# yamrom/smash-paper

Measured on AMD Instinct MI355X. Metric: reads/sec mapped+binned (hg19, 150 bp) at 1/2/4/8 MI355X; bit-exact bin counts, higher is better.
Workload: dtype u8/u64 (integer); 1 GPU; C3 hg19-shaped, 50 M x 150 bp SMASH reads per rank (25 M pairs, one run in batches), sample_bins/50000; genome=hg19, index_words=packed (SA / ISA hints, DESIGN section 3), genome_bp=3095693983, text_N=6191388016, pairs_per_rank=25000000, read_len=150, batch_pairs=12500000, bins=50000, parallelism=single GPU

## Files before the change

smash-paper_amd/csrc/mam.hip:

```cpp
#include "common.hpp"
#include "mam_device.hpp"
#include "mam_sm.hpp"

#include <algorithm>
#include <cstdio>
#include <cstdlib>
#include <vector>
#include <cstring>

namespace smash {
namespace {

template <class IdxT, int BLOCK, bool PLAIN>
__global__ __launch_bounds__(BLOCK) void k_mam(
    DevIndex<IdxT> x, const uint8_t *__restrict__ seqs, uint64_t stride,
    const uint16_t *__restrict__ lens, uint32_t len0, uint64_t n_reads,
    uint32_t min_len, uint64_t *__restrict__ out, uint32_t cap,
    uint32_t *__restrict__ n_out, uint32_t row, unsigned long long *work) {
  extern __shared__ uint8_t lds[];
  uint8_t *P = lds + threadIdx.x * row;
  for (;;) {
    const uint64_t r = atomicAdd(work, 1ull);
    if (r >= n_reads) break;
    const uint32_t L = lens ? lens[r] : len0;
// ... 77 lines not shown
    SMASH_HIP(hipMemcpy(ws, c.wave_stats, 128 * 8, hipMemcpyDeviceToHost));
    SMASH_HIP(hipFree(c.iters));
    SMASH_HIP(hipFree(c.wave_stats));
    std::vector<uint32_t> srt(hv);
    std::sort(srt.begin(), srt.end());
    double sum = 0;
    for (uint32_t v : hv) sum += v;
    auto q = [&](double f) { return srt[std::min<size_t>(srt.size() - 1, size_t(f * srt.size()))]; };
    std::fprintf(stderr,
                 "[k_mam_sm] reads %llu blocks %llu (%d/CU) row %u words: lane-iterations/read mean %.1f "
                 "p50 %u p90 %u p99 %u p99.9 %u max %u; wave-iterations %llu, active lanes/iteration %.2f\n",
                 (unsigned long long)n_reads, (unsigned long long)blocks, per_cu, c.w_row, sum / n_reads,
                 q(0.5), q(0.9), q(0.99), q(0.999), srt.back(), ws[0],
                 double(ws[1]) / double(ws[0] ? ws[0] : 1));
    static const char *names[] = {"EXIT", "NEW", "ALU", "COPY", "BM", "KT", "IDX", "BYTE", "CMP",
                                  "USCAN", "EXL", "EXR", "EXB"};
    static const char *idx_ops[] = {"SAPOS", "SAPOS2", "SCAN_SA", "ISAJ", "NS_SA2", "NS_ISA2",
                                    "TD_SA2", "TD_SA"};
    static const char *byte_ops[] = {"TD_T2", "TD_T", "LM"};
    std::fprintf(stderr, "[k_mam_sm] lane-iterations per read by state:");
    for (int k = 0; k < 13; ++k)
      if (ws[2 + k]) std::fprintf(stderr, " %s %.1f", names[k], double(ws[2 + k]) / n_reads);
    for (int k = 0; k < 8; ++k)
      if (ws[18 + k]) std::fprintf(stderr, " IDX.%s %.1f", idx_ops[k], double(ws[18 + k]) / n_reads);
    for (int k = 0; k < 3; ++k)
      if (ws[34 + k]) std::fprintf(stderr, " BYTE.%s %.1f", byte_ops[k], double(ws[34 + k]) / n_reads);
    for (int k = 0; k < 2; ++k)
      if (ws[42 + k]) std::fprintf(stderr, " CMP.%s %.1f", k ? "SCAN" : "EXT", double(ws[42 + k]) / n_reads);
    std::fprintf(stderr, "\n");
    static const char *regions[] = {
        "consume", "S_ALU", "S_COPY", "S_BM", "S_KT", "S_IDX", "S_BYTE", "S_CMP", "S_USCAN",
        "S_EX", "A_BS", "A_BS_DONE", "A_XL_DONE", "A_RUN_DONE", "A_CHAIN_DONE", "A_EXPAND",
        "A_AFTER", "A_TOP", "A_TRAV", "A_DONE", "TOP.!clean", "TOP.codes1", "TOP.codes2",
        "TOP.kt", "TOP.filter", "TOP.kcache", "dma", "rowbad"};
    std::fprintf(stderr, "[k_mam_sm] wave iterations running each region (%%):");
    for (int k = 0; k < 28; ++k)
      if (ws[64 + k])
        std::fprintf(stderr, " %s %.1f", regions[k], 100.0 * double(ws[64 + k]) / double(ws[0] ? ws[0] : 1));
    std::fprintf(stderr, "\n");
  }
  return SMASH_OK;
}

template <class IdxT>
int launch_sm(const smash_index *ix, uint32_t min_len, const uint8_t *seqs,
              uint64_t stride, const uint16_t *lens, uint32_t len,
              uint64_t n_reads, uint64_t *out, uint32_t cap, uint32_t *n_out,
              hipStream_t s, bool sync_check, const SearchWs *ws) {
  constexpr int B = kSmBlock;
  const uint32_t glen = !lens ? len : ws && ws->geom_len ? ws->geom_len : 255u;
  const sm::Geom g = sm::make_geom(glen);
  const bool direct = !lens && search_direct(seqs, stride, len);
  const uint64_t need = direct ? 0 : n_reads * g.chunks * 16;
  uint32_t *rec = ws ? reinterpret_cast<uint32_t *>(ws->rec) : nullptr;
  if (ws && need > ws->rec_bytes) {
    set_error("k_mam_sm: search workspace too small");
    return SMASH_ERR_ARG;
  }
  if (!ws && need > ix->rec_bytes) {
    SMASH_HIP(hipStreamSynchronize(s));
    if (ix->d_rec) SMASH_HIP(hipFree(ix->d_rec));
    ix->d_rec = nullptr;
    ix->rec_bytes = 0;
    const uint64_t bytes = need + need / 4;
    SMASH_HIP(hipMalloc(&ix->d_rec, bytes));
    ix->rec_bytes = bytes;
  }
  if (!ws) rec = ix->d_rec;
  const uint32_t ga = sm::prep_groups(glen);
// ... 217 lines not shown
```

smash-paper_amd/csrc/mam_sm.hpp:

```cpp
#pragma once
#include "mam_device.hpp"

#ifndef PAD_KEEP
#define PAD_KEEP(x) asm volatile("" : "+v"(x))
#endif
#ifndef SM_KNOB
#define SM_KNOB(field, dflt) (dflt)
#endif
#ifndef SM_HOOK_BM
#define SM_HOOK_BM(mode, a1, a2)
#endif
#ifndef SM_HOOK_F
#define SM_HOOK_F(j, bits)
#endif
#ifndef SM_HOOK_BS
#define SM_HOOK_BS(size, depth)
#endif
#ifndef SM_HOOK_CMPBS
#define SM_HOOK_CMPBS(begin, sp, off)
#endif
#ifndef SM_HOOK_RUN
#define SM_HOOK_RUN(begin, kind, ext_l, ext_r)
#endif
#ifndef SM_HOOK_BYTE
#define SM_HOOK_BYTE(pos)
#endif
#ifndef SM_HOOK_PARK
#define SM_HOOK_PARK(a)
#endif
#ifndef SM_LOAD16
#define SM_LOAD16(a) ::smash::sm::load16u(a)
#endif
#ifndef SM_LOAD16ST
#define SM_LOAD16ST(a, st) SM_LOAD16(a)
#endif
#ifndef SM_LOADPF16
#define SM_LOADPF16(a) ::smash::sm::load16u(a)
#endif
#ifndef SM_LOADIDX
#define SM_LOADIDX(p, i) uint64_t((p)[i])
#endif
#ifndef SM_HOOK_PF
#define SM_HOOK_PF(a)
#endif
#ifndef SM_PERM
#define SM_PERM(s0, s1, sel) __builtin_amdgcn_perm(s0, s1, sel)
#endif

#define SM_REGION(k)                                                              \
  do {                                                                            \
    if (STATS) {                                                                  \
      const uint64_t am_ = __ballot(1);                                           \
      if (lane == uint32_t(__builtin_ctzll(am_))) atomicAdd(c.wave_stats + 64 + (k), 1ull); \
    }                                                                             \
  } while (0)

#ifndef SM_DMA_ROW
#define SM_DMA_ROW(dst, src, n, lane) ::smash::sm::dma_row(dst, src, n, lane)
#endif

namespace smash {
namespace sm {

#ifdef SM_DMA_ROW_HOST
__device__ __forceinline__ uint4 load16u(uint64_t a) {
  uint4 v;
  __builtin_memcpy(&v, reinterpret_cast<const uint8_t *>(a), 16);
  return v;
}
#else
typedef uint32_t sm_u32x4 __attribute__((ext_vector_type(4)));
typedef sm_u32x4 sm_u32x4_u __attribute__((aligned(1)));
typedef __attribute__((address_space(1))) const sm_u32x4_u glb_block16_t;
__device__ __forceinline__ uint4 load16u(uint64_t a) {
  const sm_u32x4 b = *reinterpret_cast<glb_block16_t *>(a);
  return make_uint4(b.x, b.y, b.z, b.w);
}
#endif

#ifndef SM_DMA_ROW_HOST
typedef __attribute__((address_space(3))) void lds_void_t;
typedef __attribute__((address_space(1))) const void glb_void_t;
__device__ __forceinline__ void dma_row(uint32_t *dst, const uint4 *src, uint32_t n, uint32_t lane) {
  if (lane < n)
    __builtin_amdgcn_global_load_lds((glb_void_t *)(src + lane), (lds_void_t *)dst, 16, 0, 0);
}
#endif

// ... 143 lines not shown
        const uint32_t b = (w >> (8 * j)) & 0xFF;
        const bool live = i0 + j < L;
        if (!live) w &= ~(0xFFu << (8 * j));
        const uint32_t good = (b == 'a' ? ia : 0u) | (b == 'c' ? ic : 0u) |
                              (b == 'g' ? ig : 0u) | (b == 't' ? iu : 0u);
        bw |= uint32_t(live && !good) << (4 * k + j);
      }
      w8[k] = 8 * gi + k < g.w_raw ? w : 0u;
    }
  }
  o[gi] = bw;
  uint32_t *raw = o + 4 * g.c_bad;
  if (8 * gi + 8 <= g.w_row) {
    reinterpret_cast<uint4 *>(raw + 8 * gi)[0] = make_uint4(w8[0], w8[1], w8[2], w8[3]);
    reinterpret_cast<uint4 *>(raw + 8 * gi)[1] = make_uint4(w8[4], w8[5], w8[6], w8[7]);
  } else {
#pragma unroll
    for (uint32_t k = 0; k < 8; ++k)
      if (8 * gi + k < g.w_row) raw[8 * gi + k] = w8[k];
  }
  if (gi == ga - 1) {
    for (uint32_t k = ga; k < 4 * g.c_bad; ++k) o[k] = 0;
    for (uint32_t k = 8 * ga; k < g.w_row; ++k) raw[k] = 0;
  }
}

inline uint32_t prep_groups(uint32_t max_len) { return (max_len + 31) / 32; }

enum : uint32_t { S_EXIT = 0, S_NEW, S_ALU, S_COPY, S_BM, S_KT, S_IDX, S_BYTE, S_CMP, S_USCAN,
                  S_EXL, S_EXR, S_EXB };
enum : uint32_t { O_SAPOS, O_SAPOS2, O_BS_SA, O_ISAJ, O_NS_SA2, O_NS_ISA2 };
enum : uint32_t { O_EXT = 0, O_BS };
enum : uint32_t { A_NONE = 0, A_BSP, A_BS, A_BS_DONE, A_XL_DONE, A_RUN_DONE, A_CHAIN_DONE,
                  A_EXPAND, A_AFTER, A_TOP, A_TRAV, A_DONE, A_EMIT, A_EXS };
enum : uint32_t { BS_INSERT = 0, BS_LEFT, BS_RIGHT };

__device__ __forceinline__ uint64_t lo64(const uint4 &v) { return uint64_t(v.x) | (uint64_t(v.y) << 32); }
__device__ __forceinline__ uint64_t hi64(const uint4 &v) { return uint64_t(v.z) | (uint64_t(v.w) << 32); }
__device__ __forceinline__ uint32_t dword_at(const uint4 &v, uint32_t i) {
  return i == 0 ? v.x : i == 1 ? v.y : i == 2 ? v.z : v.w;
}
__device__ __forceinline__ uint32_t byte_at(const uint4 &v, uint32_t o) {
  return (dword_at(v, o >> 2) >> (8 * (o & 3))) & 0xFF;
}
__device__ __forceinline__ uint64_t bytes8_at(const uint4 &v, uint32_t o) {
  const uint64_t lo = lo64(v), hi = hi64(v);
  if (o == 0) return lo;
  if (o < 8) return (lo >> (8 * o)) | (hi << (64 - 8 * o));
  if (o == 8) return hi;
  return hi >> (8 * (o - 8));
}
__device__ __forceinline__ uint32_t agree_block(const uint4 &v, uint32_t o, const uint8_t *P,
                                                uint32_t poff, uint32_t lim) {
  uint32_t k = agree8(bytes8_at(v, o), lds_load8(P, poff), lim < 8 ? lim : 8u);
  if (k == 8 && lim > 8) k += agree8(bytes8_at(v, o + 8), lds_load8(P, poff + 8), lim - 8);
  return k;
}
template <class F>
__device__ __forceinline__ uint32_t byte_mask(const uint4 &v, F f) {
  uint32_t m = 0;
#pragma unroll
  for (uint32_t i = 0; i < 16; ++i) {
    const uint32_t b = (dword_at(v, i >> 2) >> (8 * (i & 3))) & 0xFF;
    m |= uint32_t(f(b, i)) << i;
  }
  return m;
}
// ... 192 lines not shown
}

#ifndef SM_GEO_WPS
#define SM_GEO_WPS 1
#endif
template <class IdxT, int BLOCK, bool CHECK, bool STATS, bool PK = false, int GEO = 0>
__global__ __launch_bounds__(BLOCK, GEO ? SM_GEO_WPS : 1) void k_mam_sm(const Ctx<IdxT> c) {
  static_assert(GEO == 0 || (GEO >= 21 && GEO <= 255), "GEO is 0 or the read length");
  const uint32_t gK = GEO ? 16u : c.K, gMin = GEO ? 20u : c.min_len, gB = GEO ? 18u : c.B;
  const uint32_t gRow = GEO ? geo_row(GEO) : c.w_row, gLen0 = GEO ? uint32_t(GEO) : c.len0;
  const uint32_t gDirect = GEO ? 1u : c.direct, gPad = GEO ? 0u : c.pad, gMh = GEO ? 1u : c.mhint;
  const uint32_t gLogN = GEO ? 33u : c.logN, gCap = GEO ? uint32_t(GEO) - 19u : c.cap;
  const uint16_t *const gLens = GEO ? nullptr : c.lens;
  static_assert(!PK || sizeof(IdxT) == 8, "packed words are 8-byte elements");
  constexpr uint64_t PM = PK ? kPkPosMask : ~0ull;
  extern __shared__ uint32_t ldsw[];
  const uint64_t it0 = c.in_text[0], it1 = c.in_text[1], it2 = c.in_text[2], it3 = c.in_text[3];
  auto in_text = [&](uint32_t b) {
    const uint64_t w = b < 64 ? it0 : b < 128 ? it1 : b < 192 ? it2 : it3;
    return ((w >> (b & 63)) & 1ull) != 0;
  };
  const uint64_t N = c.N;
  uint32_t *row = ldsw + threadIdx.x * gRow;
  const uint8_t *P = reinterpret_cast<const uint8_t *>(row);
  const uint32_t lane = threadIdx.x & 63;
  const uint32_t row_live = 4 * lane < gLen0 ? (gLen0 - 4 * lane < 4 ? gLen0 - 4 * lane : 4u) : 0u;

  uint64_t q_next = 0, q_end = 0;
  uint32_t st = S_NEW, op = 0, pend = A_NONE;
  uint64_t addr = 0, addr2 = 0;
  uint32_t fl = 0;
  FlagRef need2{fl, 0};
  uint64_t rd = 0;
  uint32_t L = 0, nem = 0;
  Bad bad{0, 0, 0, 0, 0, 0, 0, 0};
  uint32_t prefix = 0, depth = 0;
  uint64_t start = 0, end = 0, pos = 0;
  FlagRef have_pos{fl, 1};
  uint64_t lo = 0, hi = 0, bpos = 0, sp = 0, m = 0, bi = 0, es = 0, ee = 0;
  uint64_t &c0 = bpos, &c1 = sp;
  uint32_t lL = 0, lR = 0, best = 0, lc = 0, cbase = 0, cap = 0, bsm = 0, nblk = 0;
  FlagRef hit{fl, 2}, bm2{fl, 3}, skip_f{fl, 4}, xrun{fl, 5};
  FlagRef rdone{fl, 6};
  uint32_t fm = 0;
  uint32_t fk = 0, kp = 0, fj = 0, kx = 0xFFFFFFFFu;
  uint64_t klo = 1, khi = 0;
  FlagRef fdead{fl, 11};
  FlagRef ktr_set{fl, 7};
  FlagRef clean{fl, 8};
  FlagRef pf{fl, 9}, pfr{fl, 10};
  FlagRef xls{fl, 12}, xl1{fl, 13}, xrs{fl, 14}, xr1{fl, 15};
  FlagRef em{fl, 16};
  uint32_t dch = 0, j = 0, thresh = 0, xd = 0;
  uint32_t it = 0;
  uint64_t w_iters = 0, w_active = 0;
  auto uscan_start = [&](uint64_t p, uint32_t d) {
    dch = d; j = 1;
    addr = reinterpret_cast<uint64_t>(c.U + p + 1);
    addr2 = addr + 16;
    need2 = SM_KNOB(u32, 1u) && d - 1 > 16;
    st = S_USCAN;
  };
  auto bs_decide = [&](bool ranout, uint32_t pb, uint32_t tb) {
    bool left;
    if (bsm == BS_INSERT) {
      left = ranout || int8_t(pb) < int8_t(tb);
      if (lc > best) { best = lc; bpos = sp; bi = m; }
    } else {
      left = (lc >= cap) == (bsm == BS_LEFT);
    }
    if (left) { hi = m; lR = lc; }
    else { lo = m + 1; lL = lc; }
  };
  auto bs_probe = [&]() -> bool {
    SM_HOOK_CMPBS(true, sp, cbase + lc);
    const uint32_t o = cbase + lc;
    if (PK && ((sp >> kPkPosBits) & 7u) != 5u && o - gK < kPkWindow) {
      const uint32_t rem = cap - lc, nav = gK + kPkWindow - o;
      const uint32_t lim = rem < nav ? rem : nav;
      const uint64_t win = pk_window(sp) >> (8 * (o - gK));
      const uint32_t k = agree8(win, lds_load8(P, prefix + o), lim);
      lc += k;
      if (k < lim || k == rem) {
        SM_HOOK_CMPBS(false, sp, cbase + lc);
        bs_decide(k == rem, k == rem ? 0u : uint32_t(P[prefix + o + k]),
                  uint32_t(win >> (8 * (k & 7))) & 0xFFu);
        pf = false; pfr = false; need2 = false;
        return true;
      }
    }
    addr = reinterpret_cast<uint64_t>(c.T + (sp & PM) + cbase + lc);
    addr2 = ia(c.SA, (lo + m) >> 1);
    need2 = SM_KNOB(pf, 1u) && lo < m;
    pfr = SM_KNOB(pf, 1u) && m + 1 < hi;
    pf = SM_KNOB(pf, 1u) != 0;
    st = S_CMP; op = O_BS;
    return false;
  };
  auto lblock = [&](uint64_t e) { return reinterpret_cast<uint64_t>(c.L8 + (e >= 15 ? e - 15 : 0)); };
  auto ex_start = [&](uint64_t lb, uint64_t hb, bool ls, bool rs) {
    const bool l = !ls && es > lb, r = !rs && ee < hb;
    nblk = 0;
    rdone = !r;
    addr = l ? lblock(es) : reinterpret_cast<uint64_t>(c.L8 + ee + 1);
    addr2 = reinterpret_cast<uint64_t>(c.L8 + ee + 1);
    need2 = l && r;
    st = l && r ? S_EXB : l ? S_EXL : S_EXR;
    return l || r;
  };

  auto isa_hints = [&](uint64_t wl, uint64_t wr) {
    const uint32_t d = depth;
    xls = pk_below(wl, 40, d) || (pk_above(wl, 40, d) && pk_below(wl, 33, d));
    xl1 = !pk_below(wl, 40, d);
    xrs = pk_below(wr, 47, d) || (pk_above(wr, 47, d) && pk_below(wr, 54, d));
    xr1 = !pk_below(wr, 47, d);
  };

  for (;;) {
    const uint64_t newm = __ballot(st == S_NEW);
    const uint32_t need = uint32_t(__popcll(newm));
    const uint64_t avail = q_end - q_next;
    const uint64_t live = __ballot(st != S_EXIT);
    if (live == 0) break;
    if (STATS) { w_iters += 1; w_active += __popcll(live); }
    const uint32_t st_ld = S_COPY + gDirect;
    if (CHECK && st >= st_ld &&
        (addr < c.lo || addr >= c.hi || (need2 && (addr2 < c.lo || addr2 >= c.hi)))) {
      if (atomicAdd(c.viol, 1ull) == 0) {
        c.viol[1] = st; c.viol[2] = op; c.viol[3] = addr; c.viol[4] = need2 ? addr2 : 0;
// ... 42 lines not shown
          cm &= cm - 1;
          const uint32_t w = row_live ? ldsw[ln * gRow + lane] : 0u;
          const uint32_t nib = row_live ? bad_nibble(w, c.bad_tab_lo, c.bad_tab_hi, row_live) : 0u;
          if (__ballot(nib != 0)) {
            uint32_t x = nib << (4 * (lane & 7));
            x |= __shfl_xor(x, 1, 64);
            x |= __shfl_xor(x, 2, 64);
            x |= __shfl_xor(x, 4, 64);
            const uint32_t m0 = __shfl(x, 0, 64), m1 = __shfl(x, 8, 64), m2 = __shfl(x, 16, 64),
                           m3 = __shfl(x, 24, 64), m4 = __shfl(x, 32, 64), m5 = __shfl(x, 40, 64),
                           m6 = __shfl(x, 48, 64), m7 = __shfl(x, 56, 64);
            if (lane == ln) bad = Bad{m0, m1, m2, m3, m4, m5, m6, m7};
          }
        }
#endif
      }
    }
    bool fresh = false;
    if (newm) {
      if (take) base = __shfl(base, int(__builtin_ctzll(newm)), 64);
      if (st == S_NEW) {
        fresh = true;
        const uint32_t r = uint32_t(__popcll(newm & ((1ull << lane) - 1)));
        rd = r < avail ? q_next + r : base + (r - avail);
        if (rd >= c.n_reads) {
          st = S_EXIT;
        } else {
          L = gLens ? gLens[rd] : gLen0;
          addr = reinterpret_cast<uint64_t>(c.rec + rd * c.chunks);
          addr2 = addr + 16;
          need2 = !gDirect && c.c_bad > 1;
          pf = false; pfr = false;
          bad = Bad{0, 0, 0, 0, 0, 0, 0, 0};
          st = S_COPY;
        }
      }
      if (take) { q_next = base + (need - avail); q_end = base + take; }
      else q_next += need;
      uint64_t fm_ = __ballot(fresh && st == S_COPY);
      if (fm_) SM_REGION(26);
      while (fm_) {
        const uint32_t ln = uint32_t(__builtin_ctzll(fm_));
        fm_ &= fm_ - 1;
        const uint64_t rl = __shfl(rd, int(ln), 64);
        if (gDirect)
          SM_DMA_ROW(ldsw + ln * gRow, c.rows + rl * (gRow >> 2), gRow >> 2, lane);
        else
          SM_DMA_ROW(ldsw + ln * gRow, c.rec + rl * c.chunks + c.c_bad, c.chunks - c.c_bad, lane);
      }
    }
    if (st < S_ALU || fresh) continue;
    if (STATS) {
      ++it;
      atomicAdd(c.wave_stats + 2 + (st == S_IDX ? 16 + op : st == S_CMP ? 40 + op : st), 1ull);
    }
#ifdef SM_TRACE
    if (st != S_COPY)
      printf("it %u st %u op %u prefix %u depth %u [%llu,%llu] pos %llu hp %d\n", it, st, op, prefix,
             depth, (unsigned long long)start, (unsigned long long)end, (unsigned long long)pos,
             int(have_pos));
#endif
    const uint32_t ao = st >= S_BYTE ? 0u : uint32_t(addr) & 15;
    uint32_t a = A_NONE;
    SM_REGION(0);
    uint32_t mv = 0, mv2 = 0;
    if (st >= S_USCAN) {
      const bool us = st == S_USCAN;
      const uint32_t base = us ? dch - j - 1 : xd - 1;
      mv = thr_mask(v, base, us);
      mv2 = thr_mask(v2, us ? base - 16 : base, us);
    }

    switch (st) {
      case S_ALU:
        SM_REGION(1);
        a = pend;
        break;
      case S_COPY: {
        SM_REGION(2);
        if (!gDirect) {
          bad.w0 = v.x; bad.w1 = v.y; bad.w2 = v.z; bad.w3 = v.w;
          bad.w4 = v2.x; bad.w5 = v2.y; bad.w6 = v2.z; bad.w7 = v2.w;
        }
        need2 = false;
        prefix = 0; depth = 0; start = 0; end = N - 1; have_pos = false; nem = 0;
        skip_f = false; fm = 0; ktr_set = false;
        fk = 0; kp = 0; kx = 0xFFFFFFFFu; fdead = false;
        clean = (bad.w0 | bad.w1 | bad.w2 | bad.w3 | bad.w4 | bad.w5 | bad.w6 | bad.w7) == 0;
        a = A_TOP;
        break;
      }
      case S_BM: {
        SM_REGION(3);
        const bool two = need2;
        need2 = false;
        if (SM_KNOB(bm_dual, 3u) == 3) {
          const uint32_t nb = 2 * (gK + 4);
          auto entry_bits = [&](const uint4 &e, uint64_t cc) {
            const uint64_t f48 = kt_filter(lo64(e), hi64(e));
            const uint32_t l1 = uint32_t(cc >> (nb - 2)) & 3, l0 = uint32_t(cc >> (nb - 4)) & 3;
            const uint32_t r1 = uint32_t(cc >> 2) & 3, r2 = uint32_t(cc) & 3;
            return (uint32_t(f48 >> (32 + 4 * l1 + l0)) & 1u) |
                   ((uint32_t(f48 >> (16 + 4 * l0 + r1)) & 1u) << 1) |
                   ((uint32_t(f48 >> (4 * r1 + r2)) & 1u) << 2);
          };
          const uint32_t bits = entry_bits(v, c0);
          SM_HOOK_F(fj, bits);
          fk |= (7u << fj) | (bits << (16 + fj));
          fdead = bits != 7u;
          if (two) {
            const uint32_t bits2 = entry_bits(v2, c1);
            SM_HOOK_F(fj + 3, bits2);
            fk |= (7u << (fj + 3)) | (bits2 << (19 + fj));
            fdead = fdead || bits2 != 7u;
          }
          kx = kp + fj + 2;
          klo = lo64(v) & kKtMask;
          khi = hi64(v) & kKtMask;
          a = A_TOP;
          break;
        }
        const uint64_t cc = bm2 ? c0 : c1;
        const bool pa = (lo64(v) >> (40 + (cc & 15))) & 1ull;
        const bool pb = !SM_KNOB(bm_dual, 3u) || ((lo64(v2) >> (40 + (c0 & 15))) & 1ull);
        if (SM_KNOB(bm_dual, 3u) == 2) {
          const uint32_t D = gMin - gB;
          const uint32_t fm0 = fm;
          SM_HOOK_BM(fm, pa, pb);
          uint32_t adv = 0, nfm = 0;
          bool pass = false;
          if (fm == 0) {
            if (!pa) { adv = D + 1; nfm = 1; }
            else if (!pb) adv = 1;
            else pass = true;
          } else if (fm == 1) {
            if (!pa && !pb) { adv = 2 * D + 2; nfm = 1; }
            else if (!pa) { adv = D + 1; nfm = 2; }
            else nfm = 2;
          } else {
            if (!pb) adv = 2;
            else if (!pa) adv = 1;
            else pass = true;
          }
          if (pass) {
            skip_f = true; fm = 1;
            m = (fm0 == 0 ? c0 : c1) >> (2 * (gB - gK));
            ktr_set = true;
          } else {
            fm = nfm;
            if (adv) { depth = 0; start = 0; end = N - 1; have_pos = false; prefix += adv; }
          }
          a = A_TOP;
        } else if (!pa && !bm2) {
          depth = 0; start = 0; end = N - 1; have_pos = false;
          prefix += gMin - gB + 1;
          a = A_TOP;
        } else if (!pa || !pb) {
          depth = 0; start = 0; end = N - 1; have_pos = false; ++prefix; a = A_TOP;
        } else if (!bm2 && !SM_KNOB(bm_dual, 3u)) {
          bm2 = true;
          addr = reinterpret_cast<uint64_t>(c.KT + 2 * (c0 >> 4));
        } else {
          skip_f = true;
          a = A_TOP;
        }
        break;
      }
      case S_KT: {
        SM_REGION(4);
        const uint64_t l0 = lo64(v) & kKtMask, h0 = hi64(v) & kKtMask;
        if (l0 <= h0) { depth = gK; start = l0; end = h0; have_pos = false; }
        a = A_TRAV;
        break;
      }
      case S_IDX: {
        SM_REGION(5);
        const uint64_t iv = idx_val<IdxT>(v, ao);
        const uint64_t iv2 = idx_val<IdxT>(v2, uint32_t(addr2) & 15);
        if (PK && (op == O_ISAJ || op == O_NS_ISA2)) isa_hints(iv, op == O_ISAJ ? iv : iv2);
        if (op == O_SAPOS || op == O_SAPOS2) {
          pos = iv; have_pos = true;
          a = op == O_SAPOS ? A_TRAV : A_AFTER;
        } else if (op == O_BS_SA) {
          sp = iv;
          a = A_BSP;
        } else if (op == O_ISAJ) {
          start = end = iv & PM; have_pos = false;
          a = A_EXPAND;
        } else if (op == O_NS_SA2) {
          addr = ia(c.ISA, (iv & PM) + 1); addr2 = ia(c.ISA, (iv2 & PM) + 1);
          op = O_NS_ISA2;
        } else {
          start = iv & PM; end = iv2 & PM; need2 = false;
          ++prefix; have_pos = false;
          if (depth == 0) { start = 0; end = N - 1; a = A_TOP; }
          else a = A_EXPAND;
        }
        break;
      }
      case S_BYTE: {
        SM_REGION(6);
        SM_HOOK_BYTE(pos & PM);
        em = P[prefix - 1] != uint8_t(byte_at(v, ao));
        a = A_EMIT;
        break;
      }
      case S_CMP: {
        SM_REGION(7);
        const bool tn2 = need2 && !pf;
        const uint32_t off = prefix + (op == O_BS ? cbase : depth) + lc;
        const uint32_t rem = op == O_BS ? cap - lc : L - off;
        const uint32_t lim = rem < 16 ? rem : 16u;
        uint32_t k = agree_block(v, 0, P, off, lim);
        if (tn2 && k == lim && k < rem) {
          const uint32_t lim2 = rem - k < 16 ? rem - k : 16u;
          k += agree_block(v2, 0, P, off + k, lim2);
        }
        const uint32_t got = tn2 ? (rem < 32 ? rem : 32u) : lim;
        const bool had_pf = pf;
        pf = false; pfr = false;
        lc += k;
        if (k == got && k < rem) {
          addr += k;
          addr2 = addr + 16;
          need2 = rem - k > 16;
        } else if (op == O_EXT) {
          need2 = false;
          depth += lc; lc = 0;
          a = A_AFTER;
        } else {
          SM_HOOK_CMPBS(false, sp, cbase + lc);
          need2 = false;
          const uint32_t tbyte = k < 16 ? byte_at(v, k) : byte_at(v2, k - 16);
          bs_decide(k == rem, k == rem ? 0u : uint32_t(P[off + k]), tbyte);
          const bool left = hi == m;
          if (had_pf && lo < hi) {
            m = (lo + hi) >> 1;
            SM_HOOK_PF(ia(c.SA, m));
            sp = left ? idx_val<IdxT>(v2, uint32_t(m * sizeof(IdxT)) & 15) : v3;
            lc = lL < lR ? lL : lR;
            a = A_BSP;
          } else {
            a = A_BS;
          }
        }
        break;
      }
      case S_USCAN: {
        SM_REGION(8);
        bool fin = false;
#pragma unroll
        for (uint32_t h = 0; h < 2; ++h) {
          if (fin || (h == 1 && !need2)) break;
          const uint32_t D = dch - j;
          const uint32_t lim = D < 16 ? D : 16u;
          const uint32_t inr = (1u << lim) - 1;
          const uint32_t hm = (h ? mv2 : mv) & inr;
          if (hm) {
            j += uint32_t(__builtin_ctz(hm)); hit = true; fin = true;
          } else {
            j += lim;
            if (j >= dch) { hit = false; fin = true; }
          }
        }
        if (fin) {
          need2 = false;
          a = A_CHAIN_DONE;
        } else {
          addr += need2 ? 32 : 16;
          addr2 = addr + 16;
          need2 = SM_KNOB(u32, 1u) && dch - j > 16;
        }
        break;
      }
      case S_EXL:
      case S_EXR:
      case S_EXB: {
        SM_REGION(9);
        const uint64_t lb = xrun ? start : 0, hb = xrun ? end : N - 1;
        auto side = [&](uint32_t mask, uint32_t o, bool left, bool &more) {
          const uint64_t room = left ? es - lb : hb - ee;
          const uint32_t w = left ? o + 1 : 16 - o;
          const uint32_t lim = room < uint64_t(w) ? uint32_t(room) : w;
          const uint32_t below = ~mask & 0xFFFFu;
          const uint32_t win = left ? (((1u << lim) - 1) << (o + 1 - lim)) : (((1u << lim) - 1) << o);
          const uint32_t sm = below & win;
          const uint32_t k = sm ? (left ? o - (31 - __builtin_clz(sm)) : uint32_t(__builtin_ctz(sm)) - o)
                                : lim;
          more = !sm && uint64_t(k) < room;
          return k;
        };
        bool moreL = false, moreR = false;
        if (st != S_EXR)
          es -= side(mv, uint32_t(es - (addr - reinterpret_cast<uint64_t>(c.L8))), true, moreL);
        if (st != S_EXL) {
          const bool b2 = st == S_EXB;
          ee += side(b2 ? mv2 : mv, 0u, false, moreR);
          if (b2) rdone = !moreR;
        }
        need2 = false;
        const bool left = st != S_EXR;
        const bool more = left ? moreL : moreR;
        if (!more) {
          a = left ? A_XL_DONE : A_RUN_DONE;
        } else if (++nblk < SM_KNOB(lin_blocks, 8u)) {
          addr = left ? lblock(es) : reinterpret_cast<uint64_t>(c.L8 + ee + 1);
          st = left ? S_EXL : S_EXR;
        } else {
          bsm = left ? BS_LEFT : BS_RIGHT;
          if (left) { lo = lb; hi = es; lL = 0; lR = cap; }
          else { lo = ee + 1; hi = hb + 1; lL = cap; lR = 0; }
          a = A_BS;
        }
        break;
      }
      default:
        break;
    }

    if (gPad) {
      uint32_t x = uint32_t(addr);
      for (uint32_t k = 0; k < gPad; ++k) {
        x += k;
        PAD_KEEP(x);
      }
    }

    if (a == A_BSP) {
      a = bs_probe() ? A_BS : A_NONE;
    }
    if (a == A_BS) {
      SM_REGION(10);
      if (lo < hi) {
        m = (lo + hi) >> 1;
        lc = lL < lR ? lL : lR;
        addr = ia(c.SA, m);
        st = S_IDX; op = O_BS_SA;
        a = A_NONE;
      } else {
        a = A_BS_DONE;
      }
    }
    if (a == A_BS_DONE) {
      SM_REGION(11);
      lc = 0;
      if (bsm == BS_LEFT) {
        es = lo;
        a = A_XL_DONE;
      } else if (bsm == BS_RIGHT) {
        ee = lo - 1;
        a = A_RUN_DONE;
      } else if (best == 0) {
        a = A_AFTER;
      } else {
        xd = depth + best; xrun = true;
        cbase = depth; cap = best;
        es = bi; ee = bi;
        SM_HOOK_RUN(true, 1, 0, 0);
        xls = PK && pk_below(bpos, 36, xd); xrs = PK && pk_below(bpos, 43, xd);
        a = A_EXS;
      }
    }
    if (a == A_EXPAND) {
      SM_REGION(15);
      thresh = 2u * depth * gLogN;
      xd = depth; xrun = false;
      cbase = 0; cap = depth;
      es = start; ee = end;
      SM_HOOK_RUN(true, 0, 0, 0);
      if (PK) {
        if (xls && xl1) es = start - 1;
        if (xrs && xr1) ee = end + 1;
      }
      a = A_EXS;
    }
    if (a == A_EXS) {
      a = ex_start(xrun ? start : 0, xrun ? end : N - 1, xls, xrs) ? A_NONE : A_RUN_DONE;
    }
    if (a == A_XL_DONE) {
      SM_REGION(12);
      const uint64_t hb = xrun ? end : N - 1;
      nblk = 0;
      if (!xrun && start - es >= thresh) {
        SM_HOOK_RUN(false, 0, start - es, 99);
        depth = 0; start = 0; end = N - 1; have_pos = false;
        a = A_TOP;
      } else if (ee < hb && !rdone) {
        addr = reinterpret_cast<uint64_t>(c.L8 + ee + 1);
        st = S_EXR;
        a = A_NONE;
      } else {
        a = A_RUN_DONE;
      }
    }
    if (a == A_RUN_DONE) {
      SM_REGION(13);
      SM_HOOK_RUN(false, xrun ? 1 : 0, xrun ? bi - es : start - es, xrun ? ee - bi : ee - end);
      if (xrun) {
        start = es; end = ee; depth = xd; pos = bpos; have_pos = start == end;
        a = A_AFTER;
      } else if ((start - es) + (ee - end) >= thresh) {
        depth = 0; start = 0; end = N - 1; have_pos = false;
        a = A_TOP;
      } else {
        start = es; end = ee;
        a = A_TOP;
      }
    }
    if (a == A_CHAIN_DONE) {
      SM_REGION(14);
      prefix += j;
      if (!hit) {
        depth = 0; start = 0; end = N - 1; have_pos = false;
        a = A_TOP;
      } else {
        depth = dch - j;
        addr = ia(c.ISA, (pos & PM) + j);
        st = S_IDX; op = O_ISAJ;
        a = A_NONE;
      }
    }
    if (a == A_TOP) {
      SM_REGION(17);
      uint32_t kpos = ~0u;
      const uint32_t bp0 = prefix;
      uint64_t bwin = 0;
      if (!clean) bwin = bad.bits64(prefix);
      auto badw = [&](uint32_t p, uint32_t n) {
        return uint32_t(bwin >> (p - bp0)) & ((1u << n) - 1u);
      };
      bool proceed = skip_f || depth >= gMin;
      const bool ktr = skip_f && ktr_set;
      skip_f = false; ktr_set = false;
      if (prefix >= L || (!proceed && prefix + gMin > L)) {
        a = A_DONE;
      } else if (!proceed) {
        SM_REGION(24);
        int32_t kb = -1;
        const uint32_t B = gB;
        const uint32_t D = gMin - B;
        if (!clean) {
          SM_REGION(20);
          kb = bad.last(prefix, gMin);
          while (kb >= 0 && in_text(P[kb]))
            kb = bad.last(prefix, uint32_t(kb) - prefix);
        }
        if (kb >= 0) {
          depth = 0; start = 0; end = N - 1; have_pos = false;
          prefix = uint32_t(kb) + 1;
          fm = 0;
        } else if (SM_KNOB(bm_dual, 3u) == 3) {
          if (B != gK + 2 || B > gMin || D + 3 > 16) {
            proceed = true;
          } else {
            const uint32_t sh = prefix - kp;
            uint32_t kn = sh < 16 ? (fk & 0xFFFFu) >> sh : 0u;
// ... 85 lines not shown
          if (kx == prefix) {
            SM_REGION(25);
            if (klo <= khi) { depth = gK; start = klo; end = khi; have_pos = false; }
            a = A_TRAV;
          } else {
            SM_REGION(23);
            if (ktr) addr = reinterpret_cast<uint64_t>(c.KT + 2 * m);
            else kpos = prefix;
            st = S_KT;
            a = A_NONE;
          }
        } else {
          a = A_TRAV;
        }
      }
      if (kpos != ~0u) {
        const uint64_t kmask = (1ull << (2 * gK)) - 1;
        const uint64_t cw = codes_raw7(row, gRow, kpos, gK + 7);
        const bool fb = st == S_BM;
        if (fb) {
          c0 = cw >> 6;
          c1 = cw & ((1ull << (2 * (gK + 4))) - 1);
          addr2 = reinterpret_cast<uint64_t>(c.KT + 2 * ((c1 >> 4) & kmask));
        }
        addr = reinterpret_cast<uint64_t>(c.KT + 2 * ((cw >> (fb ? 10 : 14)) & kmask));
      }
    }
    if (a == A_TRAV) {
      SM_REGION(18);
      if (depth >= L || prefix + depth >= L) {
        a = A_AFTER;
      } else {
        a = A_NONE;
        if (start == end) {
          if (!have_pos) {
            addr = ia(c.SA, start);
            st = S_IDX; op = O_SAPOS;
          } else {
            addr = reinterpret_cast<uint64_t>(c.T + (pos & PM) + depth);
            addr2 = addr + 16;
            need2 = L - prefix - depth > 16;
            st = S_CMP; op = O_EXT; lc = 0;
          }
        } else {
          SM_HOOK_BS(end - start + 1, depth);
          lo = start; hi = end + 1; lL = 0; lR = 0; best = 0;
          bsm = BS_INSERT; cbase = depth; cap = L - prefix - depth;
          m = (lo + hi) >> 1;
          lc = 0;
          addr = ia(c.SA, m);
          st = S_IDX; op = O_BS_SA;
        }
      }
    }
    if (a == A_AFTER) {
      SM_REGION(16);
      if (depth <= 1) {
        depth = 0; start = 0; end = N - 1; have_pos = false; ++prefix;
        a = A_TOP;
      } else {
        a = A_NONE;
        if (start != end) {
          --depth;
          addr = ia(c.SA, start); addr2 = ia(c.SA, end); need2 = true;
          st = S_IDX; op = O_NS_SA2;
        } else if (!have_pos) {
          addr = ia(c.SA, start);
          st = S_IDX; op = O_SAPOS2;
        } else if (depth >= gMin && prefix != 0 && (pos & PM) != 0 &&
                   (!PK || ((pos >> kPkPosBits) & 7u) >= 4u)) {
          addr = reinterpret_cast<uint64_t>(c.T + (pos & PM) - 1);
          st = S_BYTE;
        } else {
          em = depth >= gMin &&
               (!PK || prefix == 0 || (pos & PM) == 0 ||
                P[prefix - 1] != pk_char(uint32_t(pos >> kPkPosBits) & 3u));
          a = A_EMIT;
        }
      }
    }
    if (a == A_EMIT) {
      if (em) {
        if (nem < gCap)
          c.out[rd * gCap + nem] =
              pack_match(pos & PM, prefix, depth) | (PK && gMh ? pk_map_hint(pos) : 0ull);
        ++nem;
      }
      uscan_start(pos & PM, depth);
      a = A_NONE;
    }
    if (a == A_DONE) {
      SM_REGION(19);
      c.n_out[rd] = nem;
      if (STATS && c.iters) c.iters[rd] = it;
      it = 0;
      st = S_NEW;
    } else if (a != A_NONE) {
      SM_HOOK_PARK(a);
      pend = a;
      st = S_ALU;
    }
  }
  if (STATS && lane == 0) {
    atomicAdd(c.wave_stats, (unsigned long long)w_iters);
    atomicAdd(c.wave_stats + 1, (unsigned long long)w_active);
  }
}

}
}
```

Before: 481.9 million reads/s.

## Flatten state-machine switch into predicated blocks and unify top-reset path

Replaces the per-state switch in the wave-level search state machine with sequential if-blocks keyed on a snapshot of the state, and converts several branches (binary-search decide, S_IDX op dispatch, BS_DONE) into select-based predicated updates. Repeated search resets are routed through a new A_TOPR action handled inside the A_TOP block, and per-read resets move from S_COPY into the read-fetch path. Binary-search setup in A_TRAV is hoisted out of the branch. The aim is to cut divergent-branch overhead and duplicated code across lanes, at the cost of more unconditional ALU work per iteration. New stats regions are added for profiling.

```diff
diff --git a/smash-paper_amd/csrc/mam.hip b/smash-paper_amd/csrc/mam.hip
--- a/smash-paper_amd/csrc/mam.hip
+++ b/smash-paper_amd/csrc/mam.hip
@@ -133,9 +133,10 @@
         "consume", "S_ALU", "S_COPY", "S_BM", "S_KT", "S_IDX", "S_BYTE", "S_CMP", "S_USCAN",
         "S_EX", "A_BS", "A_BS_DONE", "A_XL_DONE", "A_RUN_DONE", "A_CHAIN_DONE", "A_EXPAND",
         "A_AFTER", "A_TOP", "A_TRAV", "A_DONE", "TOP.!clean", "TOP.codes1", "TOP.codes2",
-        "TOP.kt", "TOP.filter", "TOP.kcache", "dma", "rowbad"};
+        "TOP.kt", "TOP.filter", "TOP.kcache", "dma", "rowbad", "A_BSP", "A_EXS", "A_EMIT",
+        "TOP.reset"};
     std::fprintf(stderr, "[k_mam_sm] wave iterations running each region (%%):");
-    for (int k = 0; k < 28; ++k)
+    for (int k = 0; k < 32; ++k)
       if (ws[64 + k])
         std::fprintf(stderr, " %s %.1f", regions[k], 100.0 * double(ws[64 + k]) / double(ws[0] ? ws[0] : 1));
     std::fprintf(stderr, "\n");
diff --git a/smash-paper_amd/csrc/mam_sm.hpp b/smash-paper_amd/csrc/mam_sm.hpp
--- a/smash-paper_amd/csrc/mam_sm.hpp
+++ b/smash-paper_amd/csrc/mam_sm.hpp
@@ -47,6 +47,7 @@
 #define SM_PERM(s0, s1, sel) __builtin_amdgcn_perm(s0, s1, sel)
 #endif
 
+#ifndef SM_REGION
 #define SM_REGION(k)                                                              \
   do {                                                                            \
     if (STATS) {                                                                  \
@@ -54,6 +55,7 @@
       if (lane == uint32_t(__builtin_ctzll(am_))) atomicAdd(c.wave_stats + 64 + (k), 1ull); \
     }                                                                             \
   } while (0)
+#endif
 
 #ifndef SM_DMA_ROW
 #define SM_DMA_ROW(dst, src, n, lane) ::smash::sm::dma_row(dst, src, n, lane)
@@ -263,7 +265,8 @@
 enum : uint32_t { O_SAPOS, O_SAPOS2, O_BS_SA, O_ISAJ, O_NS_SA2, O_NS_ISA2 };
 enum : uint32_t { O_EXT = 0, O_BS };
 enum : uint32_t { A_NONE = 0, A_BSP, A_BS, A_BS_DONE, A_XL_DONE, A_RUN_DONE, A_CHAIN_DONE,
-                  A_EXPAND, A_AFTER, A_TOP, A_TRAV, A_DONE, A_EMIT, A_EXS };
+                  A_EXPAND, A_AFTER, A_TOP, A_TRAV, A_DONE, A_EMIT, A_EXS,
+                  A_TOPR };
 enum : uint32_t { BS_INSERT = 0, BS_LEFT, BS_RIGHT };
 
 __device__ __forceinline__ uint64_t lo64(const uint4 &v) { return uint64_t(v.x) | (uint64_t(v.y) << 32); }
@@ -522,7 +525,7 @@
   uint32_t fl = 0;
   FlagRef need2{fl, 0};
   uint64_t rd = 0;
-  uint32_t L = 0, nem = 0;
+  uint32_t L = GEO ? uint32_t(GEO) : 0u, nem = 0;
   Bad bad{0, 0, 0, 0, 0, 0, 0, 0};
   uint32_t prefix = 0, depth = 0;
   uint64_t start = 0, end = 0, pos = 0;
@@ -551,41 +554,45 @@
     need2 = SM_KNOB(u32, 1u) && d - 1 > 16;
     st = S_USCAN;
   };
-  auto bs_decide = [&](bool ranout, uint32_t pb, uint32_t tb) {
+  auto bs_decide = [&](bool on, bool ranout, uint32_t pb, uint32_t tb) {
     bool left;
     if (bsm == BS_INSERT) {
       left = ranout || int8_t(pb) < int8_t(tb);
-      if (lc > best) { best = lc; bpos = sp; bi = m; }
+      const bool up = on && lc > best;
+      best = up ? lc : best; bpos = up ? sp : bpos; bi = up ? m : bi;
     } else {
       left = (lc >= cap) == (bsm == BS_LEFT);
     }
-    if (left) { hi = m; lR = lc; }
-    else { lo = m + 1; lL = lc; }
+    const bool l = on && left, r = on && !left;
+    hi = l ? m : hi; lR = l ? lc : lR;
+    lo = r ? m + 1 : lo; lL = r ? lc : lL;
   };
   auto bs_probe = [&]() -> bool {
     SM_HOOK_CMPBS(true, sp, cbase + lc);
     const uint32_t o = cbase + lc;
+    bool dec = false;
     if (PK && ((sp >> kPkPosBits) & 7u) != 5u && o - gK < kPkWindow) {
       const uint32_t rem = cap - lc, nav = gK + kPkWindow - o;
       const uint32_t lim = rem < nav ? rem : nav;
       const uint64_t win = pk_window(sp) >> (8 * (o - gK));
       const uint32_t k = agree8(win, lds_load8(P, prefix + o), lim);
       lc += k;
-      if (k < lim || k == rem) {
-        SM_HOOK_CMPBS(false, sp, cbase + lc);
-        bs_decide(k == rem, k == rem ? 0u : uint32_t(P[prefix + o + k]),
-                  uint32_t(win >> (8 * (k & 7))) & 0xFFu);
-        pf = false; pfr = false; need2 = false;
-        return true;
-      }
-    }
-    addr = reinterpret_cast<uint64_t>(c.T + (sp & PM) + cbase + lc);
-    addr2 = ia(c.SA, (lo + m) >> 1);
-    need2 = SM_KNOB(pf, 1u) && lo < m;
-    pfr = SM_KNOB(pf, 1u) && m + 1 < hi;
-    pf = SM_KNOB(pf, 1u) != 0;
-    st = S_CMP; op = O_BS;
-    return false;
+      dec = k < lim || k == rem;
+      if (dec) { SM_HOOK_CMPBS(false, sp, cbase + lc); }
+      bs_decide(dec, k == rem, uint32_t(P[k == rem ? 0u : prefix + o + k]),
+                uint32_t(win >> (8 * (k & 7))) & 0xFFu);
+    }
+    if (dec) {
+      pf = false; pfr = false; need2 = false;
+    } else {
+      addr = reinterpret_cast<uint64_t>(c.T + (sp & PM) + cbase + lc);
+      addr2 = ia(c.SA, (lo + m) >> 1);
+      need2 = SM_KNOB(pf, 1u) && lo < m;
+      pfr = SM_KNOB(pf, 1u) && m + 1 < hi;
+      pf = SM_KNOB(pf, 1u) != 0;
+      st = S_CMP; op = O_BS;
+    }
+    return dec;
   };
   auto lblock = [&](uint64_t e) { return reinterpret_cast<uint64_t>(c.L8 + (e >= 15 ? e - 15 : 0)); };
   auto ex_start = [&](uint64_t lb, uint64_t hb, bool ls, bool rs) {
@@ -694,6 +701,9 @@
           need2 = !gDirect && c.c_bad > 1;
           pf = false; pfr = false;
           bad = Bad{0, 0, 0, 0, 0, 0, 0, 0};
+          prefix = 0; depth = 0; start = 0; end = N - 1; have_pos = false; nem = 0;
+          skip_f = false; fm = 0; ktr_set = false;
+          fk = 0; kp = 0; kx = 0xFFFFFFFFu; fdead = false;
           st = S_COPY;
         }
       }
@@ -733,55 +743,50 @@
       mv2 = thr_mask(v2, us ? base - 16 : base, us);
     }
 
-    switch (st) {
-      case S_ALU:
-        SM_REGION(1);
-        a = pend;
-        break;
-      case S_COPY: {
-        SM_REGION(2);
-        if (!gDirect) {
-          bad.w0 = v.x; bad.w1 = v.y; bad.w2 = v.z; bad.w3 = v.w;
-          bad.w4 = v2.x; bad.w5 = v2.y; bad.w6 = v2.z; bad.w7 = v2.w;
+    const uint32_t st0 = st;
+    if (st0 == S_ALU) {
+      SM_REGION(1);
+      a = pend;
+    }
+    if (st0 == S_COPY) {
+      SM_REGION(2);
+      if (!gDirect) {
+        bad.w0 = v.x; bad.w1 = v.y; bad.w2 = v.z; bad.w3 = v.w;
+        bad.w4 = v2.x; bad.w5 = v2.y; bad.w6 = v2.z; bad.w7 = v2.w;
+      }
+      need2 = false;
+      clean = (bad.w0 | bad.w1 | bad.w2 | bad.w3 | bad.w4 | bad.w5 | bad.w6 | bad.w7) == 0;
+      a = A_TOP;
+    }
+    if (st0 == S_BM) {
+      SM_REGION(3);
+      const bool two = need2;
+      need2 = false;
+      if (SM_KNOB(bm_dual, 3u) == 3) {
+        const uint32_t nb = 2 * (gK + 4);
+        auto entry_bits = [&](const uint4 &e, uint64_t cc) {
+          const uint64_t f48 = kt_filter(lo64(e), hi64(e));
+          const uint32_t l1 = uint32_t(cc >> (nb - 2)) & 3, l0 = uint32_t(cc >> (nb - 4)) & 3;
+          const uint32_t r1 = uint32_t(cc >> 2) & 3, r2 = uint32_t(cc) & 3;
+          return (uint32_t(f48 >> (32 + 4 * l1 + l0)) & 1u) |
+                 ((uint32_t(f48 >> (16 + 4 * l0 + r1)) & 1u) << 1) |
+                 ((uint32_t(f48 >> (4 * r1 + r2)) & 1u) << 2);
+        };
+        const uint32_t bits = entry_bits(v, c0);
+        SM_HOOK_F(fj, bits);
+        fk |= (7u << fj) | (bits << (16 + fj));
+        fdead = bits != 7u;
+        if (two) {
+          const uint32_t bits2 = entry_bits(v2, c1);
+          SM_HOOK_F(fj + 3, bits2);
+          fk |= (7u << (fj + 3)) | (bits2 << (19 + fj));
+          fdead = fdead || bits2 != 7u;
         }
-        need2 = false;
-        prefix = 0; depth = 0; start = 0; end = N - 1; have_pos = false; nem = 0;
-        skip_f = false; fm = 0; ktr_set = false;
-        fk = 0; kp = 0; kx = 0xFFFFFFFFu; fdead = false;
-        clean = (bad.w0 | bad.w1 | bad.w2 | bad.w3 | bad.w4 | bad.w5 | bad.w6 | bad.w7) == 0;
+        kx = kp + fj + 2;
+        klo = lo64(v) & kKtMask;
+        khi = hi64(v) & kKtMask;
         a = A_TOP;
-        break;
-      }
-      case S_BM: {
-        SM_REGION(3);
-        const bool two = need2;
-        need2 = false;
-        if (SM_KNOB(bm_dual, 3u) == 3) {
-          const uint32_t nb = 2 * (gK + 4);
-          auto entry_bits = [&](const uint4 &e, uint64_t cc) {
-            const uint64_t f48 = kt_filter(lo64(e), hi64(e));
-            const uint32_t l1 = uint32_t(cc >> (nb - 2)) & 3, l0 = uint32_t(cc >> (nb - 4)) & 3;
-            const uint32_t r1 = uint32_t(cc >> 2) & 3, r2 = uint32_t(cc) & 3;
-            return (uint32_t(f48 >> (32 + 4 * l1 + l0)) & 1u) |
-                   ((uint32_t(f48 >> (16 + 4 * l0 + r1)) & 1u) << 1) |
-                   ((uint32_t(f48 >> (4 * r1 + r2)) & 1u) << 2);
-          };
-          const uint32_t bits = entry_bits(v, c0);
-          SM_HOOK_F(fj, bits);
-          fk |= (7u << fj) | (bits << (16 + fj));
-          fdead = bits != 7u;
-          if (two) {
-            const uint32_t bits2 = entry_bits(v2, c1);
-            SM_HOOK_F(fj + 3, bits2);
-            fk |= (7u << (fj + 3)) | (bits2 << (19 + fj));
-            fdead = fdead || bits2 != 7u;
-          }
-          kx = kp + fj + 2;
-          klo = lo64(v) & kKtMask;
-          khi = hi64(v) & kKtMask;
-          a = A_TOP;
-          break;
-        }
+      } else {
         const uint64_t cc = bm2 ? c0 : c1;
         const bool pa = (lo64(v) >> (40 + (cc & 15))) & 1ull;
         const bool pb = !SM_KNOB(bm_dual, 3u) || ((lo64(v2) >> (40 + (c0 & 15))) & 1ull);
@@ -826,158 +831,146 @@
           skip_f = true;
           a = A_TOP;
         }
-        break;
-      }
-      case S_KT: {
-        SM_REGION(4);
-        const uint64_t l0 = lo64(v) & kKtMask, h0 = hi64(v) & kKtMask;
-        if (l0 <= h0) { depth = gK; start = l0; end = h0; have_pos = false; }
-        a = A_TRAV;
-        break;
-      }
-      case S_IDX: {
-        SM_REGION(5);
-        const uint64_t iv = idx_val<IdxT>(v, ao);
-        const uint64_t iv2 = idx_val<IdxT>(v2, uint32_t(addr2) & 15);
-        if (PK && (op == O_ISAJ || op == O_NS_ISA2)) isa_hints(iv, op == O_ISAJ ? iv : iv2);
-        if (op == O_SAPOS || op == O_SAPOS2) {
-          pos = iv; have_pos = true;
-          a = op == O_SAPOS ? A_TRAV : A_AFTER;
-        } else if (op == O_BS_SA) {
-          sp = iv;
+      }
+    }
+    if (st0 == S_KT) {
+      SM_REGION(4);
+      const uint64_t l0 = lo64(v) & kKtMask, h0 = hi64(v) & kKtMask;
+      if (l0 <= h0) { depth = gK; start = l0; end = h0; have_pos = false; }
+      a = A_TRAV;
+    }
+    if (st0 == S_IDX) {
+      SM_REGION(5);
+      const uint64_t iv = idx_val<IdxT>(v, ao);
+      const uint64_t iv2 = idx_val<IdxT>(v2, uint32_t(addr2) & 15);
+      if (PK && (op == O_ISAJ || op == O_NS_ISA2)) isa_hints(iv, op == O_ISAJ ? iv : iv2);
+      const uint32_t op0 = op;
+      const bool sap = op0 <= O_SAPOS2, bsa = op0 == O_BS_SA, isj = op0 == O_ISAJ;
+      const bool ns1 = op0 == O_NS_SA2, ns2 = op0 == O_NS_ISA2, se = isj || ns2;
+      const uint64_t p1 = iv & PM, p2 = iv2 & PM;
+      pos = sap ? iv : pos;
+      sp = bsa ? iv : sp;
+      start = se ? p1 : start;
+      end = isj ? p1 : ns2 ? p2 : end;
+      fl = sap ? fl | 2u : se ? fl & ~(2u | uint32_t(ns2)) : fl;
+      addr = ns1 ? ia(c.ISA, p1 + 1) : addr;
+      addr2 = ns1 ? ia(c.ISA, p2 + 1) : addr2;
+      op = ns1 ? uint32_t(O_NS_ISA2) : op0;
+      prefix += uint32_t(ns2);
+      constexpr uint32_t nxt = A_TRAV | (A_AFTER << 4) | (A_BSP << 8) | (A_EXPAND << 12) |
+                               (A_NONE << 16) | (A_EXPAND << 20);
+      a = (nxt >> (4 * op0)) & 15u;
+      a = ns2 && depth == 0 ? uint32_t(A_TOPR) : a;
+    }
+    if (st0 == S_BYTE) {
+      SM_REGION(6);
+      SM_HOOK_BYTE(pos & PM);
+      em = P[prefix - 1] != uint8_t(byte_at(v, ao));
+      a = A_EMIT;
+    }
+    if (st0 == S_CMP) {
+      SM_REGION(7);
+      const bool tn2 = need2 && !pf;
+      const uint32_t off = prefix + (op == O_BS ? cbase : depth) + lc;
+      const uint32_t rem = op == O_BS ? cap - lc : L - off;
+      const uint32_t lim = rem < 16 ? rem : 16u;
+      uint32_t k = agree_block(v, 0, P, off, lim);
+      if (tn2 && k == lim && k < rem) {
+        const uint32_t lim2 = rem - k < 16 ? rem - k : 16u;
+        k += agree_block(v2, 0, P, off + k, lim2);
+      }
+      const uint32_t got = tn2 ? (rem < 32 ? rem : 32u) : lim;
+      const bool had_pf = pf;
+      pf = false; pfr = false;
+      lc += k;
+      if (k == got && k < rem) {
+        addr += k;
+        addr2 = addr + 16;
+        need2 = rem - k > 16;
+      } else if (op == O_EXT) {
+        need2 = false;
+        depth += lc; lc = 0;
+        a = A_AFTER;
+      } else {
+        SM_HOOK_CMPBS(false, sp, cbase + lc);
+        need2 = false;
+        const uint32_t tbyte = k < 16 ? byte_at(v, k) : byte_at(v2, k - 16);
+        bs_decide(true, k == rem, k == rem ? 0u : uint32_t(P[off + k]), tbyte);
+        const bool left = hi == m;
+        if (had_pf && lo < hi) {
+          m = (lo + hi) >> 1;
+          SM_HOOK_PF(ia(c.SA, m));
+          sp = left ? idx_val<IdxT>(v2, uint32_t(m * sizeof(IdxT)) & 15) : v3;
+          lc = lL < lR ? lL : lR;
           a = A_BSP;
-        } else if (op == O_ISAJ) {
-          start = end = iv & PM; have_pos = false;
-          a = A_EXPAND;
-        } else if (op == O_NS_SA2) {
-          addr = ia(c.ISA, (iv & PM) + 1); addr2 = ia(c.ISA, (iv2 & PM) + 1);
-          op = O_NS_ISA2;
         } else {
-          start = iv & PM; end = iv2 & PM; need2 = false;
-          ++prefix; have_pos = false;
-          if (depth == 0) { start = 0; end = N - 1; a = A_TOP; }
-          else a = A_EXPAND;
-        }
-        break;
-      }
-      case S_BYTE: {
-        SM_REGION(6);
-        SM_HOOK_BYTE(pos & PM);
-        em = P[prefix - 1] != uint8_t(byte_at(v, ao));
-        a = A_EMIT;
-        break;
-      }
-      case S_CMP: {
-        SM_REGION(7);
-        const bool tn2 = need2 && !pf;
-        const uint32_t off = prefix + (op == O_BS ? cbase : depth) + lc;
-        const uint32_t rem = op == O_BS ? cap - lc : L - off;
-        const uint32_t lim = rem < 16 ? rem : 16u;
-        uint32_t k = agree_block(v, 0, P, off, lim);
-        if (tn2 && k == lim && k < rem) {
-          const uint32_t lim2 = rem - k < 16 ? rem - k : 16u;
-          k += agree_block(v2, 0, P, off + k, lim2);
-        }
-        const uint32_t got = tn2 ? (rem < 32 ? rem : 32u) : lim;
-        const bool had_pf = pf;
-        pf = false; pfr = false;
-        lc += k;
-        if (k == got && k < rem) {
-          addr += k;
-          addr2 = addr + 16;
-          need2 = rem - k > 16;
-        } else if (op == O_EXT) {
-          need2 = false;
-          depth += lc; lc = 0;
-          a = A_AFTER;
-        } else {
-          SM_HOOK_CMPBS(false, sp, cbase + lc);
-          need2 = false;
-          const uint32_t tbyte = k < 16 ? byte_at(v, k) : byte_at(v2, k - 16);
-          bs_decide(k == rem, k == rem ? 0u : uint32_t(P[off + k]), tbyte);
-          const bool left = hi == m;
-          if (had_pf && lo < hi) {
-            m = (lo + hi) >> 1;
-            SM_HOOK_PF(ia(c.SA, m));
-            sp = left ? idx_val<IdxT>(v2, uint32_t(m * sizeof(IdxT)) & 15) : v3;
-            lc = lL < lR ? lL : lR;
-            a = A_BSP;
-          } else {
-            a = A_BS;
-          }
-        }
-        break;
-      }
-      case S_USCAN: {
-        SM_REGION(8);
-        bool fin = false;
-#pragma unroll
-        for (uint32_t h = 0; h < 2; ++h) {
-          if (fin || (h == 1 && !need2)) break;
-          const uint32_t D = dch - j;
-          const uint32_t lim = D < 16 ? D : 16u;
-          const uint32_t inr = (1u << lim) - 1;
-          const uint32_t hm = (h ? mv2 : mv) & inr;
-          if (hm) {
-            j += uint32_t(__builtin_ctz(hm)); hit = true; fin = true;
-          } else {
-            j += lim;
-            if (j >= dch) { hit = false; fin = true; }
-          }
-        }
-        if (fin) {
-          need2 = false;
-          a = A_CHAIN_DONE;
-        } else {
-          addr += need2 ? 32 : 16;
-          addr2 = addr + 16;
-          need2 = SM_KNOB(u32, 1u) && dch - j > 16;
-        }
-        break;
-      }
-      case S_EXL:
-      case S_EXR:
-      case S_EXB: {
-        SM_REGION(9);
-        const uint64_t lb = xrun ? start : 0, hb = xrun ? end : N - 1;
-        auto side = [&](uint32_t mask, uint32_t o, bool left, bool &more) {
-          const uint64_t room = left ? es - lb : hb - ee;
-          const uint32_t w = left ? o + 1 : 16 - o;
-          const uint32_t lim = room < uint64_t(w) ? uint32_t(room) : w;
-          const uint32_t below = ~mask & 0xFFFFu;
-          const uint32_t win = left ? (((1u << lim) - 1) << (o + 1 - lim)) : (((1u << lim) - 1) << o);
-          const uint32_t sm = below & win;
-          const uint32_t k = sm ? (left ? o - (31 - __builtin_clz(sm)) : uint32_t(__builtin_ctz(sm)) - o)
-                                : lim;
-          more = !sm && uint64_t(k) < room;
-          return k;
-        };
-        bool moreL = false, moreR = false;
-        if (st != S_EXR)
-          es -= side(mv, uint32_t(es - (addr - reinterpret_cast<uint64_t>(c.L8))), true, moreL);
-        if (st != S_EXL) {
-          const bool b2 = st == S_EXB;
-          ee += side(b2 ? mv2 : mv, 0u, false, moreR);
-          if (b2) rdone = !moreR;
-        }
-        need2 = false;
-        const bool left = st != S_EXR;
-        const bool more = left ? moreL : moreR;
-        if (!more) {
-          a = left ? A_XL_DONE : A_RUN_DONE;
-        } else if (++nblk < SM_KNOB(lin_blocks, 8u)) {
-          addr = left ? lblock(es) : reinterpret_cast<uint64_t>(c.L8 + ee + 1);
-          st = left ? S_EXL : S_EXR;
-        } else {
-          bsm = left ? BS_LEFT : BS_RIGHT;
-          if (left) { lo = lb; hi = es; lL = 0; lR = cap; }
-          else { lo = ee + 1; hi = hb + 1; lL = cap; lR = 0; }
           a = A_BS;
         }
-        break;
-      }
-      default:
-        break;
+      }
+    }
+    if (st0 == S_USCAN) {
+      SM_REGION(8);
+      bool fin = false;
+#pragma unroll
+      for (uint32_t h = 0; h < 2; ++h) {
+        if (fin || (h == 1 && !need2)) break;
+        const uint32_t D = dch - j;
+        const uint32_t lim = D < 16 ? D : 16u;
+        const uint32_t inr = (1u << lim) - 1;
+        const uint32_t hm = (h ? mv2 : mv) & inr;
+        if (hm) {
+          j += uint32_t(__builtin_ctz(hm)); hit = true; fin = true;
+        } else {
+          j += lim;
+          if (j >= dch) { hit = false; fin = true; }
+        }
+      }
+      if (fin) {
+        need2 = false;
+        a = A_CHAIN_DONE;
+      } else {
+        addr += need2 ? 32 : 16;
+        addr2 = addr + 16;
+        need2 = SM_KNOB(u32, 1u) && dch - j > 16;
+      }
+    }
+    if (st0 >= S_EXL) {
+      SM_REGION(9);
+      const uint64_t lb = xrun ? start : 0, hb = xrun ? end : N - 1;
+      auto side = [&](uint32_t mask, uint32_t o, bool left, bool &more) {
+        const uint64_t room = left ? es - lb : hb - ee;
+        const uint32_t w = left ? o + 1 : 16 - o;
+        const uint32_t lim = room < uint64_t(w) ? uint32_t(room) : w;
+        const uint32_t below = ~mask & 0xFFFFu;
+        const uint32_t win = left ? (((1u << lim) - 1) << (o + 1 - lim)) : (((1u << lim) - 1) << o);
+        const uint32_t sm = below & win;
+        const uint32_t k = sm ? (left ? o - (31 - __builtin_clz(sm)) : uint32_t(__builtin_ctz(sm)) - o)
+                              : lim;
+        more = !sm && uint64_t(k) < room;
+        return k;
+      };
+      bool moreL = false, moreR = false;
+      if (st != S_EXR)
+        es -= side(mv, uint32_t(es - (addr - reinterpret_cast<uint64_t>(c.L8))), true, moreL);
+      if (st != S_EXL) {
+        const bool b2 = st == S_EXB;
+        ee += side(b2 ? mv2 : mv, 0u, false, moreR);
+        if (b2) rdone = !moreR;
+      }
+      need2 = false;
+      const bool left = st != S_EXR;
+      const bool more = left ? moreL : moreR;
+      if (!more) {
+        a = left ? A_XL_DONE : A_RUN_DONE;
+      } else if (++nblk < SM_KNOB(lin_blocks, 8u)) {
+        addr = left ? lblock(es) : reinterpret_cast<uint64_t>(c.L8 + ee + 1);
+        st = left ? S_EXL : S_EXR;
+      } else {
+        bsm = left ? BS_LEFT : BS_RIGHT;
+        if (left) { lo = lb; hi = es; lL = 0; lR = cap; }
+        else { lo = ee + 1; hi = hb + 1; lL = cap; lR = 0; }
+        a = A_BS;
+      }
     }
 
     if (gPad) {
@@ -989,6 +982,7 @@
     }
 
     if (a == A_BSP) {
+      SM_REGION(28);
       a = bs_probe() ? A_BS : A_NONE;
     }
     if (a == A_BS) {
@@ -1006,18 +1000,13 @@
     if (a == A_BS_DONE) {
       SM_REGION(11);
       lc = 0;
-      if (bsm == BS_LEFT) {
-        es = lo;
-        a = A_XL_DONE;
-      } else if (bsm == BS_RIGHT) {
-        ee = lo - 1;
-        a = A_RUN_DONE;
-      } else if (best == 0) {
-        a = A_AFTER;
-      } else {
+      const bool bl = bsm == BS_LEFT, br = bsm == BS_RIGHT, run = bsm == BS_INSERT && best != 0;
+      es = bl ? lo : run ? bi : es;
+      ee = br ? lo - 1 : run ? bi : ee;
+      a = bl ? uint32_t(A_XL_DONE) : br ? uint32_t(A_RUN_DONE) : uint32_t(A_AFTER);
+      if (run) {
         xd = depth + best; xrun = true;
         cbase = depth; cap = best;
-        es = bi; ee = bi;
         SM_HOOK_RUN(true, 1, 0, 0);
         xls = PK && pk_below(bpos, 36, xd); xrs = PK && pk_below(bpos, 43, xd);
         a = A_EXS;
@@ -1037,6 +1026,7 @@
       a = A_EXS;
     }
     if (a == A_EXS) {
+      SM_REGION(29);
       a = ex_start(xrun ? start : 0, xrun ? end : N - 1, xls, xrs) ? A_NONE : A_RUN_DONE;
     }
     if (a == A_XL_DONE) {
@@ -1045,8 +1035,7 @@
       nblk = 0;
       if (!xrun && start - es >= thresh) {
         SM_HOOK_RUN(false, 0, start - es, 99);
-        depth = 0; start = 0; end = N - 1; have_pos = false;
-        a = A_TOP;
+        a = A_TOPR;
       } else if (ee < hb && !rdone) {
         addr = reinterpret_cast<uint64_t>(c.L8 + ee + 1);
         st = S_EXR;
@@ -1061,20 +1050,16 @@
       if (xrun) {
         start = es; end = ee; depth = xd; pos = bpos; have_pos = start == end;
         a = A_AFTER;
-      } else if ((start - es) + (ee - end) >= thresh) {
-        depth = 0; start = 0; end = N - 1; have_pos = false;
-        a = A_TOP;
       } else {
+        a = (start - es) + (ee - end) >= thresh ? A_TOPR : A_TOP;
         start = es; end = ee;
-        a = A_TOP;
       }
     }
     if (a == A_CHAIN_DONE) {
       SM_REGION(14);
       prefix += j;
       if (!hit) {
-        depth = 0; start = 0; end = N - 1; have_pos = false;
-        a = A_TOP;
+        a = A_TOPR;
       } else {
         depth = dch - j;
         addr = ia(c.ISA, (pos & PM) + j);
@@ -1082,8 +1067,13 @@
         a = A_NONE;
       }
     }
-    if (a == A_TOP) {
+    if (a == A_TOP || a == A_TOPR) {
       SM_REGION(17);
+      if (a != A_TOP) {
+        SM_REGION(31);
+        depth = 0; start = 0; end = N - 1; have_pos = false;
+        a = A_TOP;
+      }
       uint32_t kpos = ~0u;
       const uint32_t bp0 = prefix;
       uint64_t bwin = 0;
@@ -1235,6 +1225,10 @@
         a = A_AFTER;
       } else {
         a = A_NONE;
+        lo = start; hi = end + 1; lL = 0; lR = 0; best = 0;
+        bsm = BS_INSERT; cbase = depth; cap = L - prefix - depth;
+        m = (lo + hi) >> 1;
+        lc = 0;
         if (start == end) {
           if (!have_pos) {
             addr = ia(c.SA, start);
@@ -1243,14 +1237,10 @@
             addr = reinterpret_cast<uint64_t>(c.T + (pos & PM) + depth);
             addr2 = addr + 16;
             need2 = L - prefix - depth > 16;
-            st = S_CMP; op = O_EXT; lc = 0;
+            st = S_CMP; op = O_EXT;
           }
         } else {
           SM_HOOK_BS(end - start + 1, depth);
-          lo = start; hi = end + 1; lL = 0; lR = 0; best = 0;
-          bsm = BS_INSERT; cbase = depth; cap = L - prefix - depth;
-          m = (lo + hi) >> 1;
-          lc = 0;
           addr = ia(c.SA, m);
           st = S_IDX; op = O_BS_SA;
         }
@@ -1259,8 +1249,8 @@
     if (a == A_AFTER) {
       SM_REGION(16);
       if (depth <= 1) {
-        depth = 0; start = 0; end = N - 1; have_pos = false; ++prefix;
-        a = A_TOP;
+        ++prefix;
+        a = A_TOPR;
       } else {
         a = A_NONE;
         if (start != end) {
@@ -1283,6 +1273,7 @@
       }
     }
     if (a == A_EMIT) {
+      SM_REGION(30);
       if (em) {
         if (nem < gCap)
           c.out[rd * gCap + nem] =
```

After: 495.7 million reads/s, median of 6. 2.9% higher.
